# wheretrue/exon-duckdb

Hardware: AMD Instinct MI355X
Metric: FASTQ records/sec into DataChunks (higher is better)
Workload: dtype u8; 1 GPU; read_fastq on 10 GB synthetic 150 bp FASTQ (332 B/record, 30120481 records), 1x MI355X, byte-range shards; bytes_per_gpu=9999999692, columns=name,description,sequence,quality_scores as duckdb::string_t + validity

## Files before the change

### exon_duckdb_amd/csrc/exg_fastq_fused.hip

```cpp
#include "exg_fastq.hpp"
#include "exg_fused_core.hpp"

namespace exg {

struct FastqFormat;
static constexpr int kFastqHalves = 3;


__device__ __forceinline__ void fastq_report_utf8(ScanWsHeader *hdr, long long out, int64_t rec_off) {
    atomicMin(&hdr->err_word, ((unsigned long long)out << 8) | EXG_PE_INVALID_UTF8);
    atomicMin(&hdr->err_off, (unsigned long long)rec_off);
}

template <int kMode, class L>
__device__ __forceinline__ void fastq_emit_half(const L &s, const FastqDev &a, ScanWsHeader *hdr, const TileCtx &c,
                                          unsigned long long halo_nl, uint32_t dev_mode, uint32_t lane,
                                          uint32_t wave, unsigned long long *__restrict__ tile_qend,
                                          uint64_t tile_index) {
    const unsigned long long P0 = a.first_line_index - halo_nl;
    const uint32_t i0 = (uint32_t)((3 - P0) & 3);
    const uint32_t i_first = (uint32_t)((3 - (P0 + c.P)) & 3);
    const unsigned long long q_before = c.P > i0 ? (c.P - i0 + 3) / 4 : 0;
    const unsigned long long n_hc = halo_nl > i0 ? (halo_nl - i0 + 3) / 4 : 0;
    const uint32_t n_rec = c.n_lines > i_first ? (c.n_lines - i_first + 3) / 4 : 0;
    const uint64_t ptr_of_e0 = a.payload_base + c.tile_off - kWin;

    if (threadIdx.x == 0 && (c.pass_base == 0 || n_rec)) {
        long long e = 0;
        if (n_rec) {
            e = (long long)c.tile_off + (int)s.nlist[4 + i_first + 4 * (n_rec - 1)] - kWin + 1;
            if ((unsigned long long)e > a.n_bytes) e = (long long)a.n_bytes;
        }
        if (c.pass_base) e |= (long long)(tile_qend[tile_index] & kFarBit);
        if constexpr (kMode != kLean) if (n_rec && s.nlist[i_first] == kNoneE) {
            const long long out0 = (long long)q_before - (long long)n_hc;
            const int e4 = s.nlist[4 + i_first];
            if ((uint64_t)((int64_t)c.tile_off + e4 - kWin) >= a.lead && out0 >= 0 &&
                ((a.flags & EXG_F_NO_STORE) || (unsigned long long)out0 < a.capacity)) {
                FarRec f;
#pragma unroll
                for (int k = 0; k < 5; k++) {
                    const uint32_t idx = i_first + k;
                    f.pos[k] = idx >= 4 ? c.half * kTile + (int32_t)s.nlist[idx] - kWin : s.prev32[idx];
                }
                f.flags = c.is_eof_tile ? 1u : 0u;
                f.out = out0;
                far_rec_of(tile_qend, a.n_bytes)[tile_index] = f;
                hdr->any_far = 1u;
                e |= (long long)kFarBit;
            }
        }
        tile_qend[tile_index] = (unsigned long long)e;
    }
    if (dev_mode >= 3) return;
    const bool no_store = (a.flags & EXG_F_NO_STORE) != 0;

    for (uint32_t jb = 0; jb < n_rec; jb += 64) {
        const uint32_t j = jb + lane;
        const long long out = (long long)(q_before + j) - (long long)n_hc;
        bool act = j < n_rec;
        int i = 0;
        if (act) {
            i = (int)(i_first + 4 * j);
            int e4 = s.nlist[4 + i];
            act = (uint64_t)((int64_t)c.tile_off + e4 - kWin) >= a.lead && out >= 0;
            if (act && !no_store && (unsigned long long)out >= a.capacity) {
                if (wave == 0) atomicOr(&hdr->flags, EXG_RF_CAPACITY);
                act = false;
            }
        }
        bool desc_valid = false;
        if (act) {
            const uint32_t q0 = s.nlist[i];
            uint4 val = make_uint4(0, 0, 0, 0);
            if (q0 == kNoneE) {
                if constexpr (kMode == kLean) {
                    if (wave == 0) {
                        tile_redo_of(tile_qend, a.n_bytes)[opaque_s((uint32_t)(tile_index / kFastqHalves))] = kRedoFar;
                        hdr->any_redo = 1u;
                    }
                }
            } else if (wave <= 1) {
                int s0 = (int)q0 + 1, e0 = s.nlist[i + 1];
                bool name_ok = s0 < e0 && ldb(s, s0) == '@';
                if (e0 > s0 && !(c.is_eof_tile && e0 == c.lim_e) && ldb(s, e0 - 1) == '\r') e0--;
                int ns = s0 + 1 < e0 ? s0 + 1 : e0;
                int sp = e0;
                for (uint32_t aa = (uint32_t)ns & ~3u; aa < (uint32_t)e0 && sp == e0; aa += 32) {
                    uint32_t w8[8];
#pragma unroll
                    for (int q = 0; q < 8; q++) w8[q] = ldw(s, aa + 4 * q);
                    uint32_t bits = 0;
#pragma unroll
                    for (int q = 0; q < 8; q++) bits |= nib4(match4(w8[q], 0x20202020u)) << (4 * q);
                    if (aa < (uint32_t)ns) bits &= 0xFFFFFFFFu << ((uint32_t)ns - aa);
                    if (bits) {
                        uint32_t pos = aa + (uint32_t)__ffs(bits) - 1;
                        if (pos < (uint32_t)e0) sp = (int)pos;
                        break;
                    }
                }
                int ds = sp < e0 ? sp + 1 : e0;
                if (wave == 0) {
                    uint32_t code = 0;
                    if (!name_ok)
                        code = EXG_PE_FASTQ_NAME_PREFIX;
                    if (code) {
                        atomicMin(&hdr->err_word, ((unsigned long long)out << 8) | code);
                        atomicMin(&hdr->err_off, (unsigned long long)((int64_t)c.tile_off + s0 - kWin));
                    }
                    val = make_string_lds(s, ns, (uint32_t)(sp - ns), ptr_of_e0);
                    if constexpr (kMode != kLean) {
                        if (c.non_ascii && !utf8_valid_lds(s, ns, sp)) fastq_report_utf8(hdr, out, (int64_t)c.tile_off + s0 - kWin);
                    }
                } else {
                    desc_valid = e0 > ds;
                    if (desc_valid) val = make_string_lds(s, ds, (uint32_t)(e0 - ds), ptr_of_e0);
                    if constexpr (kMode != kLean) {
                        if (c.non_ascii && !utf8_valid_lds(s, ds, e0)) fastq_report_utf8(hdr, out, (int64_t)c.tile_off + s0 - kWin);
                    }
                }
            } else {
                const int k = wave == 2 ? 1 : 3;
                int sk = (int)s.nlist[i + k] + 1, ek = s.nlist[i + k + 1];
                if (sk > ek) sk = ek;
                if (ek > sk && !(c.is_eof_tile && ek == c.lim_e) && ldb(s, ek - 1) == '\r') ek--;
                uint32_t code = 0;
                if (wave == 2) {
                    int s2 = (int)s.nlist[i + 2] + 1, e2 = s.nlist[i + 3];
                    if (!(s2 < e2 && ldb(s, s2) == '+')) code = EXG_PE_FASTQ_PLUS_PREFIX;
                }
                if (code) {
                    atomicMin(&hdr->err_word, ((unsigned long long)out << 8) | code);
                    atomicMin(&hdr->err_off, (unsigned long long)((int64_t)c.tile_off + (int)q0 + 1 - kWin));
                }
                val = make_string_lds(s, sk, (uint32_t)(ek - sk), ptr_of_e0);
                if constexpr (kMode != kLean) {
                    if (c.non_ascii && !utf8_valid_lds(s, sk, ek)) fastq_report_utf8(hdr, out, (int64_t)c.tile_off + (int)q0 + 1 - kWin);
                }
            }
            if (!no_store && (dev_mode != 2 || (val.x ^ val.y ^ val.z ^ val.w) == 0x9E3779B9u)) {
                exg_string_t *col = wave == 0 ? a.d_name : wave == 1 ? a.d_desc : wave == 2 ? a.d_seq : a.d_qual;
                st_stream16(reinterpret_cast<uint4 *>(col) + out, val);
            }
        }
        if (wave == 1 && !no_store) {
            unsigned long long b = __ballot(desc_valid);
            if (b) {
                long long out_base = (long long)(q_before + jb) - (long long)n_hc;
                if (out_base < 0) {
                    b >>= (unsigned long long)(-out_base);
                    out_base = 0;
                }
                if (lane == 0 && b) {
                    uint32_t sh = (uint32_t)(out_base & 63);
                    unsigned long long lo = b << sh, hi2 = sh ? b >> (64 - sh) : 0;
                    if (lo) atomicOr((unsigned long long *)&a.d_desc_valid[out_base >> 6], lo);
                    if (hi2) atomicOr((unsigned long long *)&a.d_desc_valid[(out_base >> 6) + 1], hi2);
                }
            }
        }
    }
}


struct FastqFormat {
    using Dev = FastqDev;
#ifndef EXG_FASTQ_NLCAP
#define EXG_FASTQ_NLCAP 512
#endif
    static constexpr int kNlCap = EXG_FASTQ_NLCAP;
    static constexpr bool kTabMapLean = false, kTabMapFull = false;
    static constexpr bool kBarriers = true;
    static constexpr int kHalves = kFastqHalves;
    static constexpr int kHalvesFull = kHalves;
    static constexpr int kMinWavesPerSimd = 6;
#ifndef EXG_FASTQ_WAVES_FULL
#define EXG_FASTQ_WAVES_FULL 5
#endif
    static constexpr int kMinWavesPerSimdRedo = 5;
    static constexpr int kMinWavesPerSimdFull = EXG_FASTQ_WAVES_FULL;
    __device__ static __forceinline__ uint32_t eof_extra_lines(unsigned long long total_lines) {
        return (total_lines & 3) == 3 ? 1u : 0u;
    }
    template <int kMode, class L>
    __device__ static __forceinline__ void emit_half(const L &s, const FastqDev &a, ScanWsHeader *hdr,
                                                     const TileCtx &c, unsigned long long halo_nl, uint32_t dev_mode,
                                                     uint32_t lane, uint32_t wave,
                                                     unsigned long long *__restrict__ tile_qend, uint64_t tile_index) {
        fastq_emit_half<kMode>(s, a, hdr, c, halo_nl, dev_mode, lane, wave, tile_qend, tile_index);
    }
    __device__ static __forceinline__ unsigned long long analytic_prefix(uint64_t off) {
        uint64_t k = off / 332, w = off % 332;
        return 4 * k + (w > 27) + (w > 178) + (w > 180);
    }
};

__global__ __launch_bounds__(256) void k_fastq_far(FastqDev a, const unsigned int *__restrict__ tileA, const int32_t *__restrict__ tileL,
                                                   const unsigned long long *__restrict__ tile_qend, const FarRec *__restrict__ far_rec,
                                                   ScanWsHeader *hdr, uint32_t n_halves) {
    if (!hdr->any_far) return;
    constexpr uint32_t kHalves = FastqFormat::kHalves;
    constexpr uint64_t kSuper = (uint64_t)kHalves * kTile;
    const bool no_store = (a.flags & EXG_F_NO_STORE) != 0;
    for (uint64_t x = (uint64_t)blockIdx.x * blockDim.x + threadIdx.x; x < n_halves; x += (uint64_t)gridDim.x * blockDim.x) {
        if (!(tile_qend[x] & kFarBit)) continue;
        const FarRec f = far_rec[x];
        const uint32_t st = (uint32_t)(x / kHalves);
        int64_t p[5];
        const bool resolved = far_positions<5>(f, st, kSuper, tileA, tileL, (a.flags & EXG_F_BOF) != 0, p);
        const unsigned long long out = (unsigned long long)f.out;
        uint4 z = {0, 0, 0, 0};
        if (!resolved) {
            atomicAdd(&hdr->n_unresolved, 1ull);
            atomicOr(&hdr->flags, EXG_RF_HEAD_UNRESOLVED);
            if (!no_store) {
                reinterpret_cast<uint4 *>(a.d_name)[out] = z;
                reinterpret_cast<uint4 *>(a.d_desc)[out] = z;
                reinterpret_cast<uint4 *>(a.d_seq)[out] = z;
                reinterpret_cast<uint4 *>(a.d_qual)[out] = z;
            }
            continue;
        }
        const FastqGeom g = fastq_geometry_at(a.d_in, a.n_bytes, p);
        uint32_t code = 0;
        if (!g.name_ok)
            code = EXG_PE_FASTQ_NAME_PREFIX;
        else if (!g.plus_ok)
            code = EXG_PE_FASTQ_PLUS_PREFIX;
        const uint64_t lens[4] = {g.name_e - g.s[0], g.e[0] - g.desc_s, g.e[1] - g.s[1], g.e[3] - g.s[3]};
        if (!code && (lens[0] > 0xFFFFFFFFull || lens[1] > 0xFFFFFFFFull || lens[2] > 0xFFFFFFFFull || lens[3] > 0xFFFFFFFFull))
            code = EXG_PE_FIELD_TOO_LONG;
        if (!code && tiles_non_ascii(tileA, kSuper, p[0] + 1, p[4]) &&
            !(utf8_valid_global(a.d_in, g.s[0], g.name_e) && utf8_valid_global(a.d_in, g.desc_s, g.e[0]) &&
              utf8_valid_global(a.d_in, g.s[1], g.e[1]) && utf8_valid_global(a.d_in, g.s[3], g.e[3])))
            code = EXG_PE_INVALID_UTF8;
        if (code) {
            atomicMin(&hdr->err_word, (out << 8) | code);
            atomicMin(&hdr->err_off, (unsigned long long)(p[0] + 1));
        }
        if (no_store) continue;
        const bool desc_valid = lens[1] != 0;
        reinterpret_cast<uint4 *>(a.d_name)[out] = make_string_global(a.d_in, g.s[0], lens[0], a.payload_base);
        reinterpret_cast<uint4 *>(a.d_desc)[out] = desc_valid ? make_string_global(a.d_in, g.desc_s, lens[1], a.payload_base) : z;
        reinterpret_cast<uint4 *>(a.d_seq)[out] = make_string_global(a.d_in, g.s[1], lens[2], a.payload_base);
        reinterpret_cast<uint4 *>(a.d_qual)[out] = make_string_global(a.d_in, g.s[3], lens[3], a.payload_base);
        if (desc_valid) atomicOr((unsigned long long *)&a.d_desc_valid[out >> 6], 1ull << (out & 63));
    }
}

__global__ __launch_bounds__(256) void k_fastq_finalize_fused(FastqDev a, ScanWsHeader *hdr,
                                                                const unsigned long long *__restrict__ tile_qend,
                                                                uint32_t n_tiles, exg_scan_result *res) {
    __shared__ unsigned long long s_qend;
    __shared__ int s_found;
    if (threadIdx.x == 0) {
        s_qend = 0;
        s_found = 0;
    }
    __syncthreads();
    if (!hdr->overflow) {
        for (int64_t base = (int64_t)n_tiles - 1; base >= 0; base -= 256) {
            int64_t t = base - threadIdx.x;
            unsigned long long q = t >= 0 ? tile_qend[t] & ~kFarBit : 0;
            if (q) atomicMax(&s_qend, q);
            if (q) s_found = 1;
            __syncthreads();
            if (s_found) break;
        }
    }
    __syncthreads();
    const unsigned long long last_qend = s_qend;
    if (threadIdx.x) return;
// ... 97 lines not shown
```

### exon_duckdb_amd/csrc/exg_fused_core.hpp

```cpp
#pragma once
#include "exg_fastq_ws.hpp"

#ifndef EXG_FIRST_POLL_SLEEP
#define EXG_FIRST_POLL_SLEEP 0
#endif
#ifndef EXG_POLL_SLEEP
#define EXG_POLL_SLEEP 2
#endif

namespace exg {


static constexpr int kTile = kFusedTileBytes;
static constexpr int kMaxHalves = 4;
static constexpr int kWin = kFusedWindow;
static constexpr int kThreads = 256;
static constexpr int kRows = kTile / (kThreads * 16);
static constexpr int kLdsBytes = kWin + kTile + 96;
static constexpr uint32_t kNoneE = 0xFFFFu;

static constexpr uint32_t kFlagA = 1u << 31;
static constexpr uint32_t kNonAsciiA = 1u << 30;
static constexpr uint32_t kCountA = kNonAsciiA - 1;
static constexpr unsigned long long kFlag = 1ull << 63;
static constexpr unsigned long long kVal = (1ull << 48) - 1;

template <int NL, int H, bool TABS = false>
struct FusedLdsT {
    static constexpr int kNlCap = NL;
    static constexpr bool kHasTabs = TABS;
    static constexpr int kTabRow = TABS ? kTile / 16 + 4 : 4;
    __attribute__((aligned(8))) uint16_t tabmap[TABS ? H : 1][kTabRow];
    uint8_t bytes[kLdsBytes];
    uint16_t nlist[4 + NL + 4];
    uint16_t bitmap[H][kTile / 16];
    uint32_t wtot[4];
    uint32_t wcnt[4];
    unsigned long long prefix;
    uint32_t hi_or[4];
    int32_t prev32[4];
    int32_t carry32[4];
    uint16_t carry[4];
};

template <class L>
__device__ __forceinline__ uint32_t ldw(const L &s, uint32_t e_aligned) {
    return *reinterpret_cast<const uint32_t *>(s.bytes + e_aligned);
}
template <class L>
__device__ __forceinline__ uint32_t ldb(const L &s, int e) { return s.bytes[e]; }
typedef uint32_t lds_u32u __attribute__((aligned(1)));
typedef uint32_t lds_v3u __attribute__((ext_vector_type(3), aligned(1)));
template <class L>
__device__ __forceinline__ uint32_t ldu32(const L &s, int e) {
    return *reinterpret_cast<const lds_u32u *>(s.bytes + e);
}

template <class L>
__device__ __forceinline__ uint4 make_string_lds(const L &s, int e, uint32_t len, uint64_t ptr_of_e0) {
    uint4 r;
    r.x = len;
    if (len <= EXG_INLINE_LENGTH) {
        const lds_v3u w = *reinterpret_cast<const lds_v3u *>(s.bytes + e);
        uint32_t m0 = len >= 4 ? 0xFFFFFFFFu : ((1u << (8 * len)) - 1u);
        uint32_t l1 = len > 4 ? len - 4 : 0, l2 = len > 8 ? len - 8 : 0;
        uint32_t m1 = l1 >= 4 ? 0xFFFFFFFFu : ((1u << (8 * l1)) - 1u);
        uint32_t m2 = l2 >= 4 ? 0xFFFFFFFFu : ((1u << (8 * l2)) - 1u);
        r.y = w.x & m0;
        r.z = w.y & m1;
        r.w = w.z & m2;
    } else {
        uint64_t ptr = ptr_of_e0 + (uint64_t)e;
        r.y = ldu32(s, e);
        r.z = (uint32_t)ptr;
        r.w = (uint32_t)(ptr >> 32);
    }
    return r;
}

template <class L>
__device__ inline bool utf8_valid_lds(const L &s, int b, int e) {
    int i = b;
    while (i < e) {
        const uint32_t c0 = ldb(s, i);
        if (c0 < 0x80) {
            i++;
            continue;
        }
        if (c0 >= 0xC2 && c0 <= 0xDF) {
            if (i + 1 >= e || (ldb(s, i + 1) & 0xC0) != 0x80) return false;
            i += 2;
        } else if (c0 >= 0xE0 && c0 <= 0xEF) {
            if (i + 2 >= e) return false;
            const uint32_t c1 = ldb(s, i + 1), c2 = ldb(s, i + 2);
            const uint32_t lo = c0 == 0xE0 ? 0xA0 : 0x80, hi = c0 == 0xED ? 0x9F : 0xBF;
            if (c1 < lo || c1 > hi || (c2 & 0xC0) != 0x80) return false;
            i += 3;
        } else if (c0 >= 0xF0 && c0 <= 0xF4) {
            if (i + 3 >= e) return false;
            const uint32_t c1 = ldb(s, i + 1), c2 = ldb(s, i + 2), c3 = ldb(s, i + 3);
            const uint32_t lo = c0 == 0xF0 ? 0x90 : 0x80, hi = c0 == 0xF4 ? 0x8F : 0xBF;
            if (c1 < lo || c1 > hi || (c2 & 0xC0) != 0x80 || (c3 & 0xC0) != 0x80) return false;
            i += 4;
        } else {
            return false;
        }
    }
    return true;
}
__device__ inline bool tiles_non_ascii(const unsigned int *__restrict__ tileA, uint64_t super_bytes, int64_t lo, int64_t hi) {
    if (lo < 0) lo = 0;
    if (hi < lo) return false;
    for (uint64_t t = (uint64_t)lo / super_bytes, t1 = (uint64_t)hi / super_bytes; t <= t1; t++)
        if (tileA[t] & kNonAsciiA) return true;
    return false;
}

// ... 120 lines not shown
    return sum;
}

template <int N>
__device__ inline bool far_positions(const FarRec &f, uint32_t st, uint64_t super_bytes, const unsigned int *__restrict__ tileA,
                                     const int32_t *__restrict__ tileL, bool bof, int64_t *p) {
    int need = 0;
#pragma unroll
    for (int k = 0; k < N; k++)
        if (f.pos[k] < 0 && -f.pos[k] > need) need = -f.pos[k];
    int64_t back0 = 0, back1 = 0, back2 = 0, back3 = 0;
    int found = 0;
    for (uint32_t t = st; found < need && t > 0;) {
        t--;
        uint32_t c = tileA[t] & kCountA;
        if (!c) continue;
        if (c > 4) c = 4;
        const int4 l = *reinterpret_cast<const int4 *>(tileL + (uint64_t)t * 4);
        const int64_t base = (int64_t)((uint64_t)t * super_bytes);
        const int32_t e[4] = {l.w, l.z, l.y, l.x};
#pragma unroll
        for (int q = 0; q < 4; q++) {
            if ((uint32_t)q < c && found < need) {
                const int64_t v = base + e[q];
                if (found == 0) back0 = v;
                else if (found == 1) back1 = v;
                else if (found == 2) back2 = v;
                else back3 = v;
                found++;
            }
        }
    }
    if (found < need && bof) {
        const int64_t v = -1;
        if (found == 0) back0 = v;
        else if (found == 1) back1 = v;
        else if (found == 2) back2 = v;
        else back3 = v;
        found++;
    }
    if (found < need) return false;
    const int64_t super_off = (int64_t)((uint64_t)st * super_bytes);
#pragma unroll
    for (int k = 0; k < N; k++) {
        const int32_t c = f.pos[k];
        p[k] = c >= 0 ? super_off + c : c == -1 ? back0 : c == -2 ? back1 : c == -3 ? back2 : back3;
    }
    return true;
}

struct TileCtx {
    uint64_t tile_off;
    unsigned long long P;
    uint32_t n_lines;
    int lim_e;
    bool is_eof_tile;
    bool first_of_buffer;
    bool non_ascii;
    uint32_t pass_base;
    int half;
};

enum { kLean = 0, kFullPrimary = 1, kFullRedo = 2, kFullIndex = 3 };
static constexpr unsigned int kRedoFar = 1u, kRedoDense = 2u, kRedoLast4 = 4u, kRedoUtf8 = 8u;

template <bool kBarriers = true>
__device__ __forceinline__ unsigned int *tile_redo_of(unsigned long long *tile_qend, uint64_t n_bytes) {
    return reinterpret_cast<unsigned int *>(tile_qend - fused_n_tiles(opaque_s64_if<kBarriers>(n_bytes)));
}
template <bool kBarriers = true>
__device__ __forceinline__ int32_t *tile_last4_of(unsigned long long *tile_qend, uint64_t n_bytes) {
    return reinterpret_cast<int32_t *>(tile_qend + fused_n_tiles(opaque_s64_if<kBarriers>(n_bytes)));
}
template <bool kBarriers = true>
__device__ __forceinline__ FarRec *far_rec_of(unsigned long long *tile_qend, uint64_t n_bytes) {
    return reinterpret_cast<FarRec *>(tile_qend + 3 * fused_n_tiles(opaque_s64_if<kBarriers>(n_bytes)));
}

template <class F, int kMode>
__global__ __launch_bounds__(kThreads, kMode == kLean ? F::kMinWavesPerSimd : (kMode == kFullPrimary || kMode == kFullIndex) ? F::kMinWavesPerSimdFull : F::kMinWavesPerSimdRedo) void k_fused(
    typename F::Dev a, unsigned int *__restrict__ tileA, unsigned long long *__restrict__ tileP, unsigned long long *__restrict__ tile_qend,
    ScanWsHeader *hdr, uint32_t n_super) {
    constexpr int kHalves = (kMode == kFullPrimary || kMode == kFullIndex) ? F::kHalvesFull : F::kHalves;
    using FusedLds = FusedLdsT<F::kNlCap, kHalves, (kMode == kLean ? F::kTabMapLean : F::kTabMapFull)>;
    constexpr int kNlCap = F::kNlCap;
    constexpr int kSuper = kTile * kHalves;
    constexpr bool kFull = kMode != kLean;
    constexpr bool kB = F::kBarriers;
    __shared__ __attribute__((aligned(16))) FusedLds s;
    const uint32_t tid = threadIdx.x;
    const uint32_t lane = tid & 63, wave = tid >> 6;
#ifdef EXG_DEV_PROBE
    const uint32_t dev_mode = (a.flags >> 8) & 15u;
#else
    constexpr uint32_t dev_mode = 0;
#endif
    uint32_t st;
    if constexpr (kMode == kFullRedo) {
        if (!hdr->any_redo) return;
        st = blockIdx.x;
    } else {
        if (blockIdx.x == 0) {
            if (wave == 0 && !(dev_mode >= 1 && dev_mode <= 3)) scanner_wave<kHalves * kTile>(a.d_in, a.n_bytes, tileA, tileP, n_super, lane);
            return;
        }
        st = blockIdx.x - 1;
    }
    uint32_t n_redone = 0;
    for (; kMode != kFullRedo || st < n_super; st += gridDim.x) {
    if constexpr (kMode == kFullRedo) {
        if (!tile_redo_of<kB>(tile_qend, a.n_bytes)[st]) continue;
        __syncthreads();
        n_redone++;
    }
    const uint64_t super_off = (uint64_t)st * kSuper;
    const uint8_t *__restrict__ d_in = a.d_in;
    const int64_t lim64 = (int64_t)a.n_bytes - (int64_t)super_off;
    const int lim_s = lim64 < kSuper ? (int)lim64 : kSuper;
    const bool last_super = st + 1 == n_super;

    uint4 v[kHalves * kRows];
    if (lim_s > 0) {
        const uint8_t *base = d_in + super_off;
        const uint32_t last = (((uint32_t)lim_s + 15u) & ~15u) - 16u;
#pragma unroll
        for (int j = 0; j < kHalves * kRows; j++) {
            const uint32_t rel = (uint32_t)(j * kThreads + tid) * 16;
            v[j] = ld_stream16(base + (rel < last ? rel : last));
        }
    } else {
#pragma unroll
        for (int j = 0; j < kHalves * kRows; j++) v[j] = make_uint4(0, 0, 0, 0);
    }
    uint4 wv = make_uint4(0, 0, 0, 0);
    const int64_t woff = (int64_t)super_off - kWin + (int64_t)lane * 16;
    if (wave == 3 && woff >= 0) wv = *reinterpret_cast<const uint4 *>(d_in + woff);

    uint32_t hi = 0, cnt = 0;
#pragma unroll
    for (int j = 0; j < kHalves * kRows; j++) {
        if (lim_s != kSuper && lim_s - (int)(j * kThreads + tid) * 16 <= 0) v[j] = make_uint4(0, 0, 0, 0);
        uint32_t mj = match16(v[j], 0x0A0A0A0Au);
        hi |= v[j].x | v[j].y | v[j].z | v[j].w;
        if (lim_s != kSuper) {
            int rem = lim_s - (int)(j * kThreads + tid) * 16;
            if (rem < 16) mj &= rem <= 0 ? 0u : ((1u << rem) - 1u);
        }
        s.bitmap[j / kRows][(j % kRows) * kThreads + tid] = (uint16_t)mj;
        if constexpr (FusedLds::kHasTabs) s.tabmap[j / kRows][(j % kRows) * kThreads + tid] = (uint16_t)match16(v[j], 0x09090909u);
        cnt += __popc(mj);
    }
    hi &= 0x80808080u;
    for (int o = 32; o > 0; o >>= 1) cnt += __shfl_down(cnt, o, 64);
    if (wave == 3) hi |= (wv.x | wv.y | wv.z | wv.w) & 0x80808080u;
    uint32_t any_hi = __any(hi != 0);
    if (lane == 0) {
        s.hi_or[wave] = any_hi;
        s.wcnt[wave] = cnt;
    }
    __syncthreads();
    const uint32_t n_nl_super = __builtin_amdgcn_readfirstlane(s.wcnt[0] + s.wcnt[1] + s.wcnt[2] + s.wcnt[3]);
    unsigned long long nl_before_half = 0;
    const bool non_ascii = (s.hi_or[0] | s.hi_or[1] | s.hi_or[2] | s.hi_or[3]) != 0;

    const bool analytic = dev_mode >= 1 && dev_mode <= 3;
    if constexpr (kMode != kFullRedo) {
        if (tid == 0 && !analytic)
            __hip_atomic_store(&tileA[st], kFlagA | n_nl_super | (non_ascii ? kNonAsciiA : 0u), __ATOMIC_RELAXED, __HIP_MEMORY_SCOPE_AGENT);
    }
#ifdef EXG_DEV_PROBE
    const unsigned long long t_pub = __builtin_amdgcn_s_memrealtime();
#endif
    const unsigned long long halo_nl = rfl64(hdr->halo_nl);
    if constexpr (kMode != kFullRedo) {
        if (non_ascii && tid == 0) {
            atomicOr(&hdr->flags, EXG_RF_NON_ASCII);
            if constexpr (kMode == kLean) {
                tile_redo_of<kB>(tile_qend, a.n_bytes)[opaque_s_if<kB>(st)] = kRedoUtf8;
                hdr->any_redo = 1u;
            }
        }
    }

#pragma unroll
    for (int h = 0; h < kHalves; h++) {
        const int lim_h = lim_s - h * kTile;
        if (h > 0 && lim_h <= 0) {
            if (tid == 0)
                for (int hh = h; hh < kHalves; hh++) tile_qend[(uint64_t)st * kHalves + hh] = 0;
            break;
        }
        if (h == 0) {
            if (wave == 3) {
                *reinterpret_cast<uint4 *>(s.bytes + lane * 16) = wv;
                if (lane < 4) s.nlist[lane] = (uint16_t)kNoneE;
                if constexpr (kFull) {
                    if (lane < 4) s.prev32[lane] = (int32_t)lane - 4;
                }
                uint32_t wm = woff >= 0 ? match16(wv, 0x0A0A0A0Au) : 0u;
                uint32_t wc = __popc(wm);
                uint32_t wincl = wave_incl_sum(wc);
                uint32_t W = __shfl(wincl, 63, 64);
                uint32_t r = wincl - wc;
                while (wm) {
                    uint32_t b = __ffs(wm) - 1;
                    wm &= wm - 1;
                    int slot = 4 - (int)(W - r);
                    if (slot >= 0) s.nlist[slot] = (uint16_t)(lane * 16 + b);
                    r++;
                }
                if (st == 0 && (a.flags & EXG_F_BOF) && lane == 0) s.nlist[3] = (uint16_t)(kWin - 1);
            }
        } else {
            uint4 t = make_uint4(0, 0, 0, 0);
            if (wave == 3) t = *reinterpret_cast<const uint4 *>(s.bytes + kTile + lane * 16);
            __syncthreads();
            if (wave == 3) {
                *reinterpret_cast<uint4 *>(s.bytes + lane * 16) = t;
                if constexpr (kFull) {
                    if (lane < 4) {
                        const int32_t code = s.carry32[lane], rel = code - (h * kTile - kWin);
                        s.prev32[lane] = code;
                        s.nlist[lane] = (code >= 0 && rel >= 0) ? (uint16_t)rel : (uint16_t)kNoneE;
                    }
                } else {
                    if (lane < 4) s.nlist[lane] = s.carry[lane];
                }
            }
        }
#pragma unroll
        for (int j = 0; j < kRows; j++)
            *reinterpret_cast<uint4 *>(s.bytes + kWin + (j * kThreads + tid) * 16) = v[h * kRows + j];
        uint32_t n_nl_h = 0;
        {
            unsigned long long mask = *reinterpret_cast<const unsigned long long *>(&s.bitmap[h][tid * 4]);
            uint32_t c = (uint32_t)__popcll(mask);
            uint32_t inc = wave_incl_sum(c);
            if (lane == 63) s.wtot[wave] = inc;
            __syncthreads();
            uint32_t r = inc - c + (wave > 0 ? s.wtot[0] : 0) + (wave > 1 ? s.wtot[1] : 0) + (wave > 2 ? s.wtot[2] : 0);
            n_nl_h = __builtin_amdgcn_readfirstlane(s.wtot[0] + s.wtot[1] + s.wtot[2] + s.wtot[3]);
            const uint32_t e0 = kWin + tid * 64;
            while (mask) {
                uint32_t b = (uint32_t)__ffsll((long long)mask) - 1;
                mask &= mask - 1;
                if (r < (uint32_t)kNlCap) s.nlist[4 + r] = (uint16_t)(e0 + b);
                r++;
            }
        }
        if (h == 0) {
            if (wave == 0) {
                unsigned long long pre;
                if constexpr (kMode == kFullRedo) {
                    pre = st ? ld_desc(&tileP[st]) & kVal : 0ull;
                } else if (analytic) {
                    pre = F::analytic_prefix(super_off);
                } else {
                    uint32_t polls = 0;
#ifdef EXG_DEV_PROBE
                    const unsigned long long t_in = __builtin_amdgcn_s_memrealtime();
#endif
                    pre = wait_prefix<kSuper>(d_in, a.n_bytes, tileA, tileP, st, lane, polls);
#ifdef EXG_DEV_PROBE
                    if (kMode == kLean && ((a.flags >> 12) & 1u) && lane == 0) {
                        const unsigned long long now = __builtin_amdgcn_s_memrealtime();
                        FarRec f = {};
// ... 33 lines not shown
        }
        c.n_lines = n_lines;
        if (ends_here && tid == 0) {
            hdr->total_nl = c.P + n_nl_h;
            hdr->total_lines = c.P + n_lines;
        }
        const uint64_t half_index = (uint64_t)st * kHalves + h;
        if constexpr (!kFull) {
            if (n_lines > (uint32_t)kNlCap) {
                if (tid == 0) {
                    tile_redo_of<kB>(tile_qend, a.n_bytes)[opaque_s_if<kB>(st)] = kRedoDense;
                    hdr->any_redo = 1u;
                }
                return;
            }
            if (h + 1 < kHalves && tid < 4) {
                uint32_t e = s.nlist[n_lines + tid];
                s.carry[tid] = (e != kNoneE && e >= (uint32_t)kTile) ? (uint16_t)(e - kTile) : (uint16_t)kNoneE;
            }
            if (h + 1 == kHalves || lim_s <= (h + 1) * kTile) {
                if (wave == 0) {
                    const uint32_t k = opaque_if<kB>(lane), idx = n_lines + k;
                    const uint32_t st_here = opaque_s_if<kB>(st);
                    int32_t code = -1;
                    if (k < 4) {
                        const uint32_t e = s.nlist[idx];
                        code = e != kNoneE ? h * kTile + (int32_t)e - kWin : -1;
                        tile_last4_of<kB>(tile_qend, a.n_bytes)[(uint64_t)st_here * 4 + k] = code;
                    }
                    const uint32_t need = n_nl_super < 4u ? n_nl_super : 4u;
                    if (__ballot(k < 4 && k >= 4 - need && code < 0) != 0 && k == 0) {
                        tile_redo_of<kB>(tile_qend, a.n_bytes)[st_here] = kRedoLast4;
                        hdr->any_redo = 1u;
                    }
                }
            }
            F::template emit_half<kLean>(s, a, hdr, c, halo_nl, dev_mode, lane, wave, tile_qend, half_index);
        } else {
            auto fill_list = [&](uint32_t base) {
                unsigned long long mask = *reinterpret_cast<const unsigned long long *>(&s.bitmap[h][tid * 4]);
                uint32_t cc = (uint32_t)__popcll(mask);
                uint32_t inc = wave_incl_sum(cc);
                uint32_t r = inc - cc + (wave > 0 ? s.wtot[0] : 0) + (wave > 1 ? s.wtot[1] : 0) + (wave > 2 ? s.wtot[2] : 0) - base;
                const uint32_t e0 = kWin + tid * 64;
                while (mask) {
                    uint32_t b = (uint32_t)__ffsll((long long)mask) - 1;
                    mask &= mask - 1;
                    if (r < (uint32_t)kNlCap) s.nlist[4 + r] = (uint16_t)(e0 + b);
                    r++;
                }
                if (tid == 0)
                    for (uint32_t q = n_nl_h > base ? n_nl_h : base; q < n_lines && q < base + (uint32_t)kNlCap; q++)
                        s.nlist[4 + q - base] = (uint16_t)c.lim_e;
            };
            const unsigned long long P_half = c.P;
#pragma unroll 1
            for (uint32_t base = 0;;) {
                const uint32_t m = n_lines - base < (uint32_t)kNlCap ? n_lines - base : (uint32_t)kNlCap;
                c.P = P_half + base;
                c.pass_base = base;
                c.n_lines = m;
                if (base + m >= n_lines && tid < 4) {
                    const uint32_t idx = m + tid;
                    const int32_t code = idx >= 4 ? h * kTile + (int32_t)s.nlist[idx] - kWin : s.prev32[idx];
                    s.carry32[tid] = code;
                    if (h + 1 == kHalves || lim_s <= (h + 1) * kTile) tile_last4_of<kB>(tile_qend, a.n_bytes)[(uint64_t)st * 4 + tid] = code;
                }
                F::template emit_half<(kMode == kFullIndex ? kFullIndex : kFullPrimary)>(s, a, hdr, c, halo_nl, dev_mode, lane, wave, tile_qend, half_index);
                base += m;
                if (base >= n_lines) break;
                uint16_t keep = 0;
                if (tid < 4) keep = s.nlist[m + tid];
                __syncthreads();
                if (tid < 4) {
                    s.nlist[tid] = keep;
                    s.prev32[tid] = h * kTile + (int32_t)keep - kWin;
                }
                fill_list(base);
                __syncthreads();
            }
        }
        if (h + 1 < kHalves) __syncthreads();
    }
    if constexpr (kMode != kFullRedo) break;
    }
    if constexpr (kMode == kFullRedo) {
        if (tid == 0 && n_redone) atomicAdd(&hdr->n_redo, n_redone);
    }
}


}
```

### exon_duckdb_amd/csrc/exg_vcf.hip

```cpp
#include <stdlib.h>

#include "exg_fused_core.hpp"
#include "exg_lines.hpp"

#include "exg_parse.hpp"
#include "exg_float_slow.hpp"

namespace exg {

struct VcfDev {
    const uint8_t *d_in;
    uint64_t n_bytes;
    uint64_t lead;
    uint64_t first_line_index;
    uint64_t payload_base;
    uint32_t flags;
    uint32_t pad;
    exg_string_t *d_fields[9];
    int64_t *d_pos;
    float *d_qual;
    uint64_t *d_qual_valid;
    uint64_t *d_formats_valid;
    uint64_t capacity;
    SlowLiteral *d_slow;
// ... 136 lines not shown
    return r;
}

__device__ __forceinline__ void store_validity64(uint64_t *words, unsigned long long bits, long long out_base,
                                                 uint32_t lane) {
    if (!words || !bits) return;
    if (out_base < 0) {
        bits >>= (unsigned long long)(-out_base);
        out_base = 0;
    }
    if (lane == 0 && bits) {
        uint32_t sh = (uint32_t)(out_base & 63);
        unsigned long long lo = bits << sh, hi = sh ? bits >> (64 - sh) : 0;
        if (lo) atomicOr((unsigned long long *)&words[out_base >> 6], lo);
        if (hi) atomicOr((unsigned long long *)&words[(out_base >> 6) + 1], hi);
    }
}

__device__ __forceinline__ void vcf_report(ScanWsHeader *hdr, uint32_t code, unsigned long long out, uint64_t line_off) {
    atomicMin(&hdr->err_word, (out << 8) | (code & 0x7Fu));
    atomicMin(&hdr->err_off, (unsigned long long)line_off);
}
__device__ __forceinline__ void vcf_slow_qual(ScanWsHeader *hdr, const VcfDev &a, uint64_t lit_off, uint32_t len, unsigned long long out,
                                              uint64_t line_off) {
    const unsigned int k = atomicAdd(&hdr->n_slow, 1u);
    if (k < a.slow_cap && out <= 0xFFFFFFFFull) {
        a.d_slow[k].off = lit_off;
        a.d_slow[k].len = len;
        a.d_slow[k].row = (unsigned int)out;
    } else {
        atomicOr(&hdr->flags, EXG_RF_QUAL_RANGE);
        vcf_report(hdr, EXG_PE_VCF_BAD_QUAL, out, line_off);
    }
}

template <class L>
struct LdsSrc {
    const L &s;
    uint64_t ptr_of_e0;
    const uint16_t *tabs;
    __device__ __forceinline__ uint32_t b(int e) const { return ldb(s, e); }
    __device__ __forceinline__ uint32_t u32(int e) const { return ldu32(s, e); }
    __device__ __forceinline__ void u96(int e, uint32_t *w0, uint32_t *w1, uint32_t *w2) const {
        const lds_v3u w = *reinterpret_cast<const lds_v3u *>(s.bytes + e);
        *w0 = w.x, *w1 = w.y, *w2 = w.z;
    }
    __device__ __forceinline__ unsigned long long tabs64(int e) const {
        typedef uint32_t lds_v4u __attribute__((ext_vector_type(4), aligned(1)));
        unsigned long long bits = 0;
#pragma unroll
        for (int q = 0; q < 4; q++) {
            const lds_v4u w = *reinterpret_cast<const lds_v4u *>(s.bytes + e + 16 * q);
            bits |= (unsigned long long)match16(make_uint4(w.x, w.y, w.z, w.w), 0x09090909u) << (16 * q);
        }
        return bits;
    }
    __device__ __forceinline__ bool tab_bits(int e, unsigned long long *out) const {
        if (!L::kHasTabs) return false;
        const int p = e - kWin;
        if (p < 0) return false;
        const unsigned long long *w = reinterpret_cast<const unsigned long long *>(tabs) + (p >> 6);
        const uint32_t sh = (uint32_t)p & 63u;
        const unsigned long long lo = w[0], hi = w[1];
        *out = sh ? (lo >> sh) | (hi << (64 - sh)) : lo;
        return true;
    }
    __device__ __forceinline__ uint4 str(int e, uint32_t len) const { return make_string_lds(s, e, len, ptr_of_e0); }
};

#ifndef EXG_VCF_HALVES
#define EXG_VCF_HALVES 2
#endif
static constexpr int kVcfHalves = EXG_VCF_HALVES;
struct VcfFormat {
    using Dev = VcfDev;
    static constexpr int kNlCap = 1024;
    static constexpr int kHalves = kVcfHalves;
#ifndef EXG_VCF_HALVES_FULL
#define EXG_VCF_HALVES_FULL 2
#endif
    static constexpr int kHalvesFull = EXG_VCF_HALVES_FULL;
    static constexpr bool kTabMapLean = true, kTabMapFull = false;
    static constexpr bool kBarriers = false;
#ifndef EXG_VCF_WAVES
#define EXG_VCF_WAVES 5
#endif
    static constexpr int kMinWavesPerSimd = EXG_VCF_WAVES;
#ifndef EXG_VCF_WAVES_FULL
#define EXG_VCF_WAVES_FULL 5
#endif
    static constexpr int kMinWavesPerSimdRedo = 4;
    static constexpr int kMinWavesPerSimdFull = EXG_VCF_WAVES_FULL;
    __device__ static __forceinline__ uint32_t eof_extra_lines(unsigned long long) { return 0; }
    __device__ static __forceinline__ unsigned long long analytic_prefix(uint64_t) { return 0; }

    template <int kMode, class L>
    __device__ static __forceinline__ void emit_half(const L &s, const VcfDev &a, ScanWsHeader *hdr,
                                                     const TileCtx &c, unsigned long long halo_nl, uint32_t dev_mode,
                                                     uint32_t lane, uint32_t wave,
                                                     unsigned long long *__restrict__ tile_qend, uint64_t tile_index) {
#ifdef EXG_VCF_ROTATE
        const uint32_t rot_w = (uint32_t)tile_index & 3u;
#else
        const uint32_t rot_w = 0;
#endif
        const uint32_t t_rot = (threadIdx.x - rot_w * 64u) & (uint32_t)(kThreads - 1);
        unsigned long long qend_word = 0;
        if (t_rot == 0 && (c.pass_base == 0 || c.n_lines)) {
            long long e = 0;
            if (c.n_lines) {
                e = (long long)c.tile_off + (int)s.nlist[4 + c.n_lines - 1] - kWin + 1;
                if ((unsigned long long)e > a.n_bytes) e = (long long)a.n_bytes;
            }
            if (c.pass_base) e |= (long long)(tile_qend[tile_index] & kFarBit);
            qend_word = (unsigned long long)e;
            tile_qend[tile_index] = qend_word;
        }
        if (dev_mode == 3 || dev_mode == 4) return;
        if constexpr (kMode == kFullIndex) {
            for (uint32_t jb = 0; jb < c.n_lines; jb += kThreads) {
                const uint32_t j = jb + t_rot;
                if (j >= c.n_lines) break;
                const unsigned long long row = c.P + j;
                if (row < a.nl_cap) a.d_nl_pos[row] = (unsigned long long)((long long)c.tile_off + (int)s.nlist[4 + j] - kWin);
                else hdr->overflow = 1u;
            }
            return;
        }
        const bool no_store = (a.flags & EXG_F_NO_STORE) != 0;
        const LdsSrc<L> src{s, a.payload_base + c.tile_off - kWin, s.tabmap[L::kHasTabs ? c.half : 0]};
        for (uint32_t jb = 0; jb < c.n_lines; jb += kThreads) {
            const uint32_t j = jb + t_rot;
            const long long out = (long long)(c.P + j) - (long long)halo_nl;
            bool act = j < c.n_lines;
            int e1 = 0;
            if (act) {
                e1 = s.nlist[4 + j];
                act = (uint64_t)((int64_t)c.tile_off + e1 - kWin) >= a.lead && out >= 0;
                if (act && !no_store && (unsigned long long)out >= a.capacity) {
                    atomicOr(&hdr->flags, EXG_RF_CAPACITY);
                    act = false;
                }
            }
            bool qv = false, rv = false;
            if (act) {
                const uint32_t q0 = s.nlist[3 + j];
                if (q0 == kNoneE) {
                    if constexpr (kMode == kLean) {
                        tile_redo_of<false>(tile_qend, a.n_bytes)[(uint32_t)(tile_index / kVcfHalves)] = kRedoFar;
                        hdr->any_redo = 1u;
                    } else {
                        FarRec f;
                        f.pos[0] = s.prev32[3];
                        f.pos[1] = c.half * kTile + e1 - kWin;
                        f.pos[2] = f.pos[3] = f.pos[4] = 0;
                        f.flags = c.is_eof_tile ? 1u : 0u;
                        f.out = out;
                        far_rec_of<false>(tile_qend, a.n_bytes)[tile_index] = f;
                        hdr->any_far = 1u;
                        tile_qend[tile_index] = qend_word | kFarBit;
                    }
                } else {
                    int s0 = (int)q0 + 1;
                    if (e1 > s0 && !(c.is_eof_tile && e1 == c.lim_e) && ldb(s, e1 - 1) == '\r') e1--;
#ifdef EXG_DEV_PROBE
                    if (dev_mode == 6) continue;
// ... 547 lines not shown
```

Baseline: 13.64 billion records/s.

## Build newline lists for all FASTQ halves up front with one packed scan

In the lean FASTQ path, the newline positions for all three halves of a super-tile are now ranked in one block-wide scan. A packed three-field count word carries the per-half ranks, and each half's list is written into its own LDS array. This removes the per-half list rebuild and its barrier round trips between emitting halves. In exchange it uses extra LDS for two more newline lists, which may reduce occupancy, and it adds a redo fallback when per-half counts overflow the packed fields or the list capacity.

```diff
diff --git a/exon_duckdb_amd/csrc/exg_fastq_fused.hip b/exon_duckdb_amd/csrc/exg_fastq_fused.hip
--- a/exon_duckdb_amd/csrc/exg_fastq_fused.hip
+++ b/exon_duckdb_amd/csrc/exg_fastq_fused.hip
@@ -13,7 +13,7 @@
 }
 
 template <int kMode, class L>
-__device__ __forceinline__ void fastq_emit_half(const L &s, const FastqDev &a, ScanWsHeader *hdr, const TileCtx &c,
+__device__ __forceinline__ void fastq_emit_half(const L &s, const uint16_t *nl, const FastqDev &a, ScanWsHeader *hdr, const TileCtx &c,
                                           unsigned long long halo_nl, uint32_t dev_mode, uint32_t lane,
                                           uint32_t wave, unsigned long long *__restrict__ tile_qend,
                                           uint64_t tile_index) {
@@ -28,20 +28,20 @@
     if (threadIdx.x == 0 && (c.pass_base == 0 || n_rec)) {
         long long e = 0;
         if (n_rec) {
-            e = (long long)c.tile_off + (int)s.nlist[4 + i_first + 4 * (n_rec - 1)] - kWin + 1;
+            e = (long long)c.tile_off + (int)nl[4 + i_first + 4 * (n_rec - 1)] - kWin + 1;
             if ((unsigned long long)e > a.n_bytes) e = (long long)a.n_bytes;
         }
         if (c.pass_base) e |= (long long)(tile_qend[tile_index] & kFarBit);
-        if constexpr (kMode != kLean) if (n_rec && s.nlist[i_first] == kNoneE) {
+        if constexpr (kMode != kLean) if (n_rec && nl[i_first] == kNoneE) {
             const long long out0 = (long long)q_before - (long long)n_hc;
-            const int e4 = s.nlist[4 + i_first];
+            const int e4 = nl[4 + i_first];
             if ((uint64_t)((int64_t)c.tile_off + e4 - kWin) >= a.lead && out0 >= 0 &&
                 ((a.flags & EXG_F_NO_STORE) || (unsigned long long)out0 < a.capacity)) {
                 FarRec f;
 #pragma unroll
                 for (int k = 0; k < 5; k++) {
                     const uint32_t idx = i_first + k;
-                    f.pos[k] = idx >= 4 ? c.half * kTile + (int32_t)s.nlist[idx] - kWin : s.prev32[idx];
+                    f.pos[k] = idx >= 4 ? c.half * kTile + (int32_t)nl[idx] - kWin : s.prev32[idx];
                 }
                 f.flags = c.is_eof_tile ? 1u : 0u;
                 f.out = out0;
@@ -62,7 +62,7 @@
         int i = 0;
         if (act) {
             i = (int)(i_first + 4 * j);
-            int e4 = s.nlist[4 + i];
+            int e4 = nl[4 + i];
             act = (uint64_t)((int64_t)c.tile_off + e4 - kWin) >= a.lead && out >= 0;
             if (act && !no_store && (unsigned long long)out >= a.capacity) {
                 if (wave == 0) atomicOr(&hdr->flags, EXG_RF_CAPACITY);
@@ -71,7 +71,7 @@
         }
         bool desc_valid = false;
         if (act) {
-            const uint32_t q0 = s.nlist[i];
+            const uint32_t q0 = nl[i];
             uint4 val = make_uint4(0, 0, 0, 0);
             if (q0 == kNoneE) {
                 if constexpr (kMode == kLean) {
@@ -81,7 +81,7 @@
                     }
                 }
             } else if (wave <= 1) {
-                int s0 = (int)q0 + 1, e0 = s.nlist[i + 1];
+                int s0 = (int)q0 + 1, e0 = nl[i + 1];
                 bool name_ok = s0 < e0 && ldb(s, s0) == '@';
                 if (e0 > s0 && !(c.is_eof_tile && e0 == c.lim_e) && ldb(s, e0 - 1) == '\r') e0--;
                 int ns = s0 + 1 < e0 ? s0 + 1 : e0;
@@ -122,12 +122,12 @@
                 }
             } else {
                 const int k = wave == 2 ? 1 : 3;
-                int sk = (int)s.nlist[i + k] + 1, ek = s.nlist[i + k + 1];
+                int sk = (int)nl[i + k] + 1, ek = nl[i + k + 1];
                 if (sk > ek) sk = ek;
                 if (ek > sk && !(c.is_eof_tile && ek == c.lim_e) && ldb(s, ek - 1) == '\r') ek--;
                 uint32_t code = 0;
                 if (wave == 2) {
-                    int s2 = (int)s.nlist[i + 2] + 1, e2 = s.nlist[i + 3];
+                    int s2 = (int)nl[i + 2] + 1, e2 = nl[i + 3];
                     if (!(s2 < e2 && ldb(s, s2) == '+')) code = EXG_PE_FASTQ_PLUS_PREFIX;
                 }
                 if (code) {
@@ -171,6 +171,7 @@
 #endif
     static constexpr int kNlCap = EXG_FASTQ_NLCAP;
     static constexpr bool kTabMapLean = false, kTabMapFull = false;
+    static constexpr bool kListsAhead = true;
     static constexpr bool kBarriers = true;
     static constexpr int kHalves = kFastqHalves;
     static constexpr int kHalvesFull = kHalves;
@@ -188,7 +189,14 @@
                                                      const TileCtx &c, unsigned long long halo_nl, uint32_t dev_mode,
                                                      uint32_t lane, uint32_t wave,
                                                      unsigned long long *__restrict__ tile_qend, uint64_t tile_index) {
-        fastq_emit_half<kMode>(s, a, hdr, c, halo_nl, dev_mode, lane, wave, tile_qend, tile_index);
+        fastq_emit_half<kMode>(s, s.nlist, a, hdr, c, halo_nl, dev_mode, lane, wave, tile_qend, tile_index);
+    }
+    template <int kMode, class L>
+    __device__ static __forceinline__ void emit_half_list(const L &s, const uint16_t *nl, const FastqDev &a, ScanWsHeader *hdr,
+                                                          const TileCtx &c, unsigned long long halo_nl, uint32_t dev_mode,
+                                                          uint32_t lane, uint32_t wave,
+                                                          unsigned long long *__restrict__ tile_qend, uint64_t tile_index) {
+        fastq_emit_half<kMode>(s, nl, a, hdr, c, halo_nl, dev_mode, lane, wave, tile_qend, tile_index);
     }
     __device__ static __forceinline__ unsigned long long analytic_prefix(uint64_t off) {
         uint64_t k = off / 332, w = off % 332;
diff --git a/exon_duckdb_amd/csrc/exg_fused_core.hpp b/exon_duckdb_amd/csrc/exg_fused_core.hpp
--- a/exon_duckdb_amd/csrc/exg_fused_core.hpp
+++ b/exon_duckdb_amd/csrc/exg_fused_core.hpp
@@ -25,7 +25,7 @@
 static constexpr unsigned long long kFlag = 1ull << 63;
 static constexpr unsigned long long kVal = (1ull << 48) - 1;
 
-template <int NL, int H, bool TABS = false>
+template <int NL, int H, bool TABS = false, int NLISTS = 1>
 struct FusedLdsT {
     static constexpr int kNlCap = NL;
     static constexpr bool kHasTabs = TABS;
@@ -33,6 +33,8 @@
     __attribute__((aligned(8))) uint16_t tabmap[TABS ? H : 1][kTabRow];
     uint8_t bytes[kLdsBytes];
     uint16_t nlist[4 + NL + 4];
+    uint16_t nlist_ahead[NLISTS - 1][4 + NL + 4];
+    __device__ __forceinline__ uint16_t *nlist_of(int h) { return NLISTS > 1 && h > 0 ? nlist_ahead[h - 1] : nlist; }
     uint16_t bitmap[H][kTile / 16];
     uint32_t wtot[4];
     uint32_t wcnt[4];
@@ -319,7 +321,8 @@
     typename F::Dev a, unsigned int *__restrict__ tileA, unsigned long long *__restrict__ tileP, unsigned long long *__restrict__ tile_qend,
     ScanWsHeader *hdr, uint32_t n_super) {
     constexpr int kHalves = (kMode == kFullPrimary || kMode == kFullIndex) ? F::kHalvesFull : F::kHalves;
-    using FusedLds = FusedLdsT<F::kNlCap, kHalves, (kMode == kLean ? F::kTabMapLean : F::kTabMapFull)>;
+    constexpr bool kAhead = kMode == kLean && F::kListsAhead;
+    using FusedLds = FusedLdsT<F::kNlCap, kHalves, (kMode == kLean ? F::kTabMapLean : F::kTabMapFull), (kAhead ? kHalves : 1)>;
     constexpr int kNlCap = F::kNlCap;
     constexpr int kSuper = kTile * kHalves;
     constexpr bool kFull = kMode != kLean;
@@ -419,6 +422,175 @@
         }
     }
 
+    if constexpr (kAhead) {
+    static_assert(kHalves == 3 && kNlCap < 1024, "the packed rank word has three fields, the narrowest of 10 bits");
+    constexpr uint32_t kSh1 = 10, kSh2 = 21;
+    if (wave == 3) {
+        *reinterpret_cast<uint4 *>(s.bytes + lane * 16) = wv;
+        if (lane < 4) s.nlist[lane] = (uint16_t)kNoneE;
+        uint32_t wm = woff >= 0 ? match16(wv, 0x0A0A0A0Au) : 0u;
+        uint32_t wc = __popc(wm);
+        uint32_t wincl = wave_incl_sum(wc);
+        uint32_t W = __shfl(wincl, 63, 64);
+        uint32_t r = wincl - wc;
+        while (wm) {
+            uint32_t b = __ffs(wm) - 1;
+            wm &= wm - 1;
+            int slot = 4 - (int)(W - r);
+            if (slot >= 0) s.nlist[slot] = (uint16_t)(lane * 16 + b);
+            r++;
+        }
+        if (st == 0 && (a.flags & EXG_F_BOF) && lane == 0) s.nlist[3] = (uint16_t)(kWin - 1);
+    }
+#pragma unroll
+    for (int j = 0; j < kRows; j++) *reinterpret_cast<uint4 *>(s.bytes + kWin + (j * kThreads + tid) * 16) = v[j];
+    uint32_t pk = 0;
+#pragma unroll
+    for (int h = 0; h < kHalves; h++) {
+        const unsigned long long mask = *reinterpret_cast<const unsigned long long *>(&s.bitmap[h][tid * 4]);
+        pk += (uint32_t)__popcll(mask) << (h == 0 ? 0u : h == 1 ? kSh1 : kSh2);
+    }
+    const uint32_t inc = wave_incl_sum(pk);
+    if (lane == 63) s.wtot[wave] = inc;
+    __syncthreads();
+    const uint32_t w0 = __builtin_amdgcn_readfirstlane(s.wtot[0]), w1 = __builtin_amdgcn_readfirstlane(s.wtot[1]);
+    const uint32_t w2 = __builtin_amdgcn_readfirstlane(s.wtot[2]), w3 = __builtin_amdgcn_readfirstlane(s.wtot[3]);
+    constexpr uint32_t kM0 = (1u << kSh1) - 1u, kM1 = (1u << (kSh2 - kSh1)) - 1u;
+    uint32_t n_nl_of[kHalves];
+    n_nl_of[0] = (w0 & kM0) + (w1 & kM0) + (w2 & kM0) + (w3 & kM0);
+    n_nl_of[1] = ((w0 >> kSh1) & kM1) + ((w1 >> kSh1) & kM1) + ((w2 >> kSh1) & kM1) + ((w3 >> kSh1) & kM1);
+    n_nl_of[2] = (w0 >> kSh2) + (w1 >> kSh2) + (w2 >> kSh2) + (w3 >> kSh2);
+    if (n_nl_of[0] + n_nl_of[1] + n_nl_of[2] != n_nl_super || n_nl_of[0] > (uint32_t)kNlCap || n_nl_of[1] > (uint32_t)kNlCap ||
+        n_nl_of[2] > (uint32_t)kNlCap) {
+        if (tid == 0) {
+            tile_redo_of<kB>(tile_qend, a.n_bytes)[opaque_s_if<kB>(st)] = kRedoDense;
+            hdr->any_redo = 1u;
+        }
+        return;
+    }
+    {
+        const uint32_t r = inc - pk + (wave > 0 ? w0 : 0) + (wave > 1 ? w1 : 0) + (wave > 2 ? w2 : 0);
+        const uint32_t e0 = kWin + tid * 64;
+#pragma unroll
+        for (int h = 0; h < kHalves; h++) {
+            unsigned long long mask = *reinterpret_cast<const unsigned long long *>(&s.bitmap[h][tid * 4]);
+            uint32_t rh = h == 0 ? r & kM0 : h == 1 ? (r >> kSh1) & kM1 : r >> kSh2;
+            uint16_t *nl = s.nlist_of(h);
+            while (mask) {
+                uint32_t b = (uint32_t)__ffsll((long long)mask) - 1;
+                mask &= mask - 1;
+                nl[4 + rh] = (uint16_t)(e0 + b);
+                rh++;
+            }
+        }
+    }
+#pragma unroll
+    for (int h = 0; h < kHalves; h++) {
+        const int lim_h = lim_s - h * kTile;
+        if (h > 0 && lim_h <= 0) {
+            if (tid == 0)
+                for (int hh = h; hh < kHalves; hh++) tile_qend[(uint64_t)st * kHalves + hh] = 0;
+            break;
+        }
+        if (h == 0) {
+            if (wave == 0) {
+                unsigned long long pre;
+                if (analytic) {
+                    pre = F::analytic_prefix(super_off);
+                } else {
+                    uint32_t polls = 0;
+#ifdef EXG_DEV_PROBE
+                    const unsigned long long t_in = __builtin_amdgcn_s_memrealtime();
+#endif
+                    pre = wait_prefix<kSuper>(d_in, a.n_bytes, tileA, tileP, st, lane, polls);
+#ifdef EXG_DEV_PROBE
+                    if (((a.flags >> 12) & 1u) && lane == 0) {
+                        const unsigned long long now = __builtin_amdgcn_s_memrealtime();
+                        FarRec f = {};
+                        f.pos[0] = (int32_t)(now - t_in);
+                        f.pos[1] = (int32_t)(now - t_pub);
+                        f.pos[2] = (int32_t)polls;
+                        far_rec_of<kB>(tile_qend, a.n_bytes)[(uint64_t)st * kHalves] = f;
+                    }
+#endif
+                }
+                if (lane == 0) s.prefix = pre;
+            }
+        } else {
+            __syncthreads();
+            if (wave == 3) {
+                const uint4 t = *reinterpret_cast<const uint4 *>(s.bytes + kTile + lane * 16);
+                *reinterpret_cast<uint4 *>(s.bytes + lane * 16) = t;
+            }
+#pragma unroll
+            for (int j = 0; j < kRows; j++)
+                *reinterpret_cast<uint4 *>(s.bytes + kWin + (j * kThreads + tid) * 16) = v[h * kRows + j];
+        }
+        __syncthreads();
+        uint16_t *nl = s.nlist_of(h);
+        const uint32_t n_nl_h = n_nl_of[h];
+
+        TileCtx c;
+        c.tile_off = super_off + (uint64_t)h * kTile;
+        c.P = rfl64(s.prefix) + nl_before_half;
+        nl_before_half += n_nl_h;
+        c.first_of_buffer = st == 0 && h == 0;
+        c.pass_base = 0;
+        c.half = h;
+        c.non_ascii = non_ascii;
+        const bool ends_here = last_super && lim_h <= kTile;
+        c.is_eof_tile = ends_here && (a.flags & EXG_F_EOF);
+        c.lim_e = (lim_h < kTile ? lim_h : kTile) + kWin;
+        uint32_t n_lines = n_nl_h;
+        if (c.is_eof_tile) {
+            const unsigned long long P0 = a.first_line_index - halo_nl;
+            bool unterminated = a.n_bytes > 0 && ldb(s, c.lim_e - 1) != '\n';
+            uint32_t n0 = n_lines;
+            if (unterminated) n_lines++;
+            n_lines += F::eof_extra_lines(P0 + c.P + n_lines);
+            if (tid == 0)
+                for (uint32_t q = n0; q < n_lines && q < (uint32_t)kNlCap; q++) nl[4 + q] = (uint16_t)c.lim_e;
+            __syncthreads();
+        }
+        c.n_lines = n_lines;
+        if (ends_here && tid == 0) {
+            hdr->total_nl = c.P + n_nl_h;
+            hdr->total_lines = c.P + n_lines;
+        }
+        if (n_lines > (uint32_t)kNlCap) {
+            if (tid == 0) {
+                tile_redo_of<kB>(tile_qend, a.n_bytes)[opaque_s_if<kB>(st)] = kRedoDense;
+                hdr->any_redo = 1u;
+            }
+            return;
+        }
+        if (h + 1 == kHalves || lim_s <= (h + 1) * kTile) {
+            if (wave == 0) {
+                const uint32_t k = opaque_if<kB>(lane), idx = n_lines + k;
+                const uint32_t st_here = opaque_s_if<kB>(st);
+                int32_t code = -1;
+                if (k < 4) {
+                    const uint32_t e = nl[idx];
+                    code = e != kNoneE ? h * kTile + (int32_t)e - kWin : -1;
+                    tile_last4_of<kB>(tile_qend, a.n_bytes)[(uint64_t)st_here * 4 + k] = code;
+                }
+                const uint32_t need = n_nl_super < 4u ? n_nl_super : 4u;
+                if (__ballot(k < 4 && k >= 4 - need && code < 0) != 0 && k == 0) {
+                    tile_redo_of<kB>(tile_qend, a.n_bytes)[st_here] = kRedoLast4;
+                    hdr->any_redo = 1u;
+                }
+            }
+        }
+        F::template emit_half_list<kLean>(s, nl, a, hdr, c, halo_nl, dev_mode, lane, wave, tile_qend, (uint64_t)st * kHalves + h);
+        if (h == 0 && wave == 3 && lane < 4) {
+#pragma unroll
+            for (int g = 1; g < kHalves; g++) {
+                const uint32_t e = s.nlist_of(g - 1)[n_nl_of[g - 1] + lane];
+                s.nlist_of(g)[lane] = (e != kNoneE && e >= (uint32_t)kTile) ? (uint16_t)(e - kTile) : (uint16_t)kNoneE;
+            }
+        }
+    }
+    } else {
 #pragma unroll
     for (int h = 0; h < kHalves; h++) {
         const int lim_h = lim_s - h * kTile;
@@ -618,6 +790,7 @@
         }
         if (h + 1 < kHalves) __syncthreads();
     }
+    }
     if constexpr (kMode != kFullRedo) break;
     }
     if constexpr (kMode == kFullRedo) {
diff --git a/exon_duckdb_amd/csrc/exg_vcf.hip b/exon_duckdb_amd/csrc/exg_vcf.hip
--- a/exon_duckdb_amd/csrc/exg_vcf.hip
+++ b/exon_duckdb_amd/csrc/exg_vcf.hip
@@ -242,6 +242,7 @@
     static constexpr int kHalvesFull = EXG_VCF_HALVES_FULL;
     static constexpr bool kTabMapLean = true, kTabMapFull = false;
     static constexpr bool kBarriers = false;
+    static constexpr bool kListsAhead = false;
 #ifndef EXG_VCF_WAVES
 #define EXG_VCF_WAVES 5
 #endif
```

After: 14.13 billion records/s (median of 6 runs). 3.6% higher.
